# onecodex/needletail

Measured on AMD Instinct MI355X. Metric: Gbases/s canonical k=21 on 150 bp FASTQ; % HBM-read roofline at 1/2/4/8 GPU, higher is better.
Workload: dtype u64; 1 GPU; configs[1]: synthetic FASTQ 10M x 150 bp, k=21 canonical k-mers (normalize -> reverse_complement -> canonical_kmers), reduce mode, device-resident batch; reads_total=10000000, reads_this_gpu=10000000, read_len=150, k=21, seed=0x5eed0002, outputs=n_total,n_fwd,n_rc,4096-bin prefix histogram,sum64,xor64, parallelism=single GPU, rccl_ranks=0, devices_visible=1

## Files before the change

needletail_amd/csrc/ntk_api.hip:

```cpp
#include "../../include/needletail_amd.h"

#include <hip/hip_runtime.h>
#include <rccl/rccl.h>
#include <dlfcn.h>
#include <time.h>

#include <cstdlib>
#include <cstring>
#include <map>
#include <mutex>
#include <new>
#include <utility>
#include <thread>
#include <algorithm>
#include <vector>

#include "ntk_kernels.hpp"
#include "ntk_plan.hpp"
#include "ntk_compat_plan.hpp"

using namespace ntk;

const void *ntk_pick_scan2(int k, bool tie_rc, bool accept_u);
const void *ntk_pick_scan2_q(int k, bool canonical, bool tie_rc, bool accept_u);
// ... 301 lines not shown
    if (f.rearm_shards) c->work_dirty = false;
    return NTK_OK;
}

inline bool bad_device_input(const uint8_t *d_seq, const uint8_t *d_qual) { return !d_seq || ((uintptr_t)d_seq & 15) || ((uintptr_t)d_qual & 15); }

inline void scan_args_set_quality(ScanArgs &a, const uint8_t *d_qual, uint32_t cutoff)
{
    if (!cutoff) return;
    const QualityCut qc = quality_cut(cutoff);
    a.qual = d_qual; a.q_add = qc.add; a.q_sel = qc.sel;
}
template <class KernelQ, class Kernel, class... Args>
void launch_with_quality(ntk_ctx *c, KernelQ kernel_q, Kernel kernel, int blocks, int threads, const uint8_t *d_qual, uint32_t cutoff, Args... args)
{
    if (d_qual) {
        const QualityCut qc = quality_cut(cutoff);
        hipLaunchKernelGGL(kernel_q, dim3(blocks), dim3(threads), 0, c->stream, args..., d_qual, qc.add, qc.sel);
    } else
        hipLaunchKernelGGL(kernel, dim3(blocks), dim3(threads), 0, c->stream, args...);
}

inline int raw_bytes_blocks(const ntk_ctx *c, uint64_t n) { return blocks_for(c, n, (uint64_t)kPlThreads * 32, 8); }

template <bool WIDE> constexpr auto bytes_reduce_q = &canonical_bytes_reduce_kernel<WIDE, true, const uint8_t *, uint32_t, uint32_t>;
template <bool ACCEPT_U> constexpr auto wide_reduce_q = &wide_canonical_reduce_kernel<ACCEPT_U, true, const uint8_t *, uint32_t, uint32_t>;

void launch_raw_bytes(ntk_ctx *c, bool wide, int blocks, const uint8_t *d_seq, uint64_t n, uint32_t k, const uint32_t *run_if, bool normalized,
                      const uint8_t *d_qual, uint32_t cutoff)
{
    const uint32_t pb = k < 6 ? k : 6;
    launch_with_quality(c, wide ? bytes_reduce_q<true> : bytes_reduce_q<false>, wide ? &canonical_bytes_reduce_kernel<true> : &canonical_bytes_reduce_kernel<false>,
                        blocks, kPlThreads, d_qual, cutoff, d_seq, n, (n + 15) & ~(uint64_t)15, k, 2u * (k - pb), c->lut_complement(),
                        c->d_part_hist.p, c->d_part_scalars.p, run_if, wide && normalized ? 1u : 0u);
}

int run_bytes_reduce(ntk_ctx *c, const uint8_t *d_seq, uint64_t n, const ntk_params *p, bool zero_first, bool normalized,
                     const uint8_t *d_qual, uint32_t cutoff)
{
    const bool wide = p->k > 32, packed_first = wide && !(c->route_off & NTK_ROUTE_NO_SPECULATION);
    if (zero_first) HIPCHK(hipMemsetAsync(c->d_acc, 0, NTK_ACC_WORDS * sizeof(uint64_t), c->stream));
    const int blocks_raw = raw_bytes_blocks(c, n), blocks = packed_first ? blocks_for(c, n, kWkTile, 8) : blocks_raw;
    int rc = ensure_partials(c, blocks > blocks_raw ? blocks : blocks_raw);
    if (rc) return rc;
    Fold fold;
    fold.undigested = wide;
    TimedSpan span;
    if ((rc = span.begin(c))) return rc;
    if (packed_first) {
        const FlagPair f = next_flag(c);
        launch_with_quality(c, normalized ? wide_reduce_q<true> : wide_reduce_q<false>,
                            normalized ? &wide_canonical_reduce_kernel<true> : &wide_canonical_reduce_kernel<false>, blocks, kWkThreads, d_qual, cutoff,
                            d_seq, n, p->k, c->d_part_hist.p, c->d_part_scalars.p, f.flag, f.next);
        HIPCHK(hipGetLastError());
        fold.alt_flag = f.flag; fold.alt_rows = blocks_raw;
    }
    launch_raw_bytes(c, wide, blocks_raw, d_seq, n, p->k, fold.alt_flag, normalized, d_qual, cutoff);
    HIPCHK(hipGetLastError());
    if ((rc = span.end(c->ev_used))) return rc;
    return launch_fold(c, blocks, fold);
}

struct TileScan {
    const void *fn = nullptr;
    int threads = 0;
    size_t lds = 0;
    uint32_t stride = 0;
    uint64_t max_chunk = 0;
    int max_per_cu = 0;
    bool reduce = true;
    bool speculate = false;
    uint32_t cutoff = 0;
};
int launch_tile_scan(ntk_ctx *c, const TileScan &s, ScanArgs &a, bool zero_first)
{
    int per_cu = 0, rc = resident_blocks(c, s.fn, s.threads, s.lds, s.max_per_cu, &per_cu);
    if (rc) return rc;
    const uint64_t blocks_max = block_cap(c, per_cu), waves_per_block = (uint64_t)s.threads / 64;
    const uint64_t n = a.n_bytes;
    const int blocks_raw = s.speculate ? raw_bytes_blocks(c, n) : 0;
    a.n_tiles = tile_count(n, s.stride);
    a.work_counters = c->d_work.p;
    a.zero_words = NTK_ACC_WORDS;
    for (uint64_t tb = 0; tb < a.n_tiles; tb += kMaxTilesPerLaunch) {
        const LaunchPlan lp = plan_launch(n, s.stride, tb, blocks_max, waves_per_block, s.max_chunk);
        const int blocks = (int)lp.blocks;
        a.tile_begin = lp.tile_begin; a.tile_end = lp.tile_end;
        a.tail_tile_rel = lp.tail_tile_rel;
        a.n_shards = lp.n_shards;
        a.tiles_per_shard = lp.tiles_per_shard;
        a.chunk_tiles = lp.chunk_tiles;
        a.zero_acc = zero_first ? c->d_acc : nullptr;
        zero_first = false;
        if (c->work_dirty) HIPCHK(hipMemsetAsync(c->d_work.p, 0, kMaxShards * 64, c->stream));
        c->work_dirty = true;
        if (s.reduce) {
            if ((rc = ensure_partials(c, blocks > blocks_raw ? blocks : blocks_raw))) return rc;
            a.part_hist = c->d_part_hist.p; a.part_scalars = c->d_part_scalars.p;
        }
        Fold fold;
        fold.rearm_shards = a.n_shards;
        if (s.speculate) {
            const FlagPair f = next_flag(c);
            a.lower_flag = f.flag; a.lower_flag_next = f.next;
            fold.alt_flag = f.flag; fold.alt_rows = blocks_raw;
        }
        TimedSpan span;
        if ((rc = span.begin(c))) return rc;
        void *kargs[] = {(void *)&a};
        HIPCHK(hipLaunchKernel(s.fn, dim3(blocks), dim3(s.threads), kargs, s.lds, c->stream));
        if (s.speculate) {
            launch_raw_bytes(c, false, blocks_raw, a.seq, n, a.k, fold.alt_flag, false, a.qual, s.cutoff);
            HIPCHK(hipGetLastError());
        }
        if ((rc = span.end(c->ev_used))) return rc;
        if (s.reduce && (rc = launch_fold(c, blocks, fold))) return rc;
    }
    return NTK_OK;
}

int run_scan(ntk_ctx *c, const uint8_t *d_seq, uint64_t n, const ntk_params *p, const Mode &m, bool reduce,
             uint64_t *d_values, uint16_t *d_valid16, uint16_t *d_rc16, const uint8_t *d_qual = nullptr, const void *fused_min_fn = nullptr,
             uint32_t fused_w = 0)
{
    const bool zero_first = reduce && (p->flags & NTK_FLAG_RESET);
    if (n == 0) {
        if (zero_first) HIPCHK(hipMemsetAsync(c->d_acc, 0, NTK_ACC_WORDS * sizeof(uint64_t), c->stream));
        return NTK_OK;
    }
    if (bad_device_input(d_seq, d_qual)) return NTK_ERR_BAD_ARG;
    const uint32_t cutoff = d_qual ? quality_cutoff(p) : 0u;
    const uint32_t stride = !reduce ? (uint32_t)kTileStride : (p->k <= 32 ? (uint32_t)sv2_stride_bytes((int)(fused_w ? p->k + fused_w - 1 : p->k), fused_w == 0) : 0u);
    bool speculate = false;
    if (m.raw_bytes) {
        if (p->k > 32 && (!reduce || fused_min_fn)) return NTK_ERR_BAD_K;
        if (!reduce || fused_min_fn) return NTK_ERR_UNSUPPORTED;
        const uint8_t *qual = cutoff ? d_qual : nullptr;
        speculate = p->k <= 32 && tile_count(n, stride) <= kMaxTilesPerLaunch && !(c->route_off & NTK_ROUTE_NO_SPECULATION);
        if (!speculate) return run_bytes_reduce(c, d_seq, n, p, zero_first, m.accept_u, qual, cutoff);
    }
    const void *fn = fused_min_fn ? fused_min_fn : pick_scan(m, p->k, reduce, cutoff != 0);
    if (!fn) return NTK_ERR_BAD_ARG;
    int threads = !reduce ? 256 : (c->launch_threads ? c->launch_threads : 768);
    if (reduce && !c->launch_threads) {
        auto it = c->auto_threads.find(fn);
        if (it != c->auto_threads.end()) threads = it->second;
        else {
            int best_waves = 0;
            for (int t : {768, 640, 512}) {
                int blocks_cu = 0;
                HIPCHK(hipOccupancyMaxActiveBlocksPerMultiprocessor(&blocks_cu, fn, t, 0));
                if (blocks_cu > 2) blocks_cu = 2;
                if (blocks_cu * t > best_waves) { best_waves = blocks_cu * t; threads = t; }
            }
            c->auto_threads[fn] = threads;
        }
    }
    TileScan s;
    s.fn = fn; s.threads = threads; s.stride = stride; s.max_chunk = 24;
    s.lds = reduce ? 0 : (size_t)(threads / 64) * kStageWaveU64 * sizeof(uint64_t);
    s.max_per_cu = reduce ? 2 * (1024 / threads) : 4;
    s.reduce = reduce; s.speculate = speculate; s.cutoff = cutoff;
    ScanArgs a;
    memset(&a, 0, sizeof(a));
    scan_args_set_k(a, p->k);
    a.seq = d_seq; a.n_bytes = n;
    a.values = d_values; a.valid16 = d_valid16; a.rc16 = d_rc16;
    scan_args_set_quality(a, d_qual, cutoff);
    return launch_tile_scan(c, s, a, zero_first);
}

const void *pick_min_generic(const Mode &m, bool quality, bool f64, uint32_t k)
{
    const int kw = f64 ? 2 : m.kw;
// ... 1355 lines not shown
```

needletail_amd/csrc/ntk_kernels.hpp:

```cpp
#pragma once
#include <hip/hip_runtime.h>
#include <stdint.h>
#include <type_traits>

#include "ntk_tile.hpp"

namespace ntk {

typedef uint32_t u32x4 __attribute__((ext_vector_type(4)));

constexpr int kDppWaveShr1 = 0x138;
struct DevXL {
    __device__ __forceinline__ uint32_t prev_and(int s, uint32_t x, uint32_t mask) const { return prev(s, x) & mask; }
    __device__ __forceinline__ uint32_t prev_auto(uint32_t x) const { return prev(0, x); }
    __device__ __forceinline__ uint32_t prev(int, uint32_t x) const
    {
        return (uint32_t)__builtin_amdgcn_mov_dpp((int)x, kDppWaveShr1, 0xf, 0xf, true);
    }
    __device__ __forceinline__ uint32_t prev_add(int, uint32_t x, uint32_t c) const
    {
        uint32_t r;
        asm("s_nop 1\n v_add_u32_dpp %0, %1, %2 wave_shr:1 row_mask:0xf bank_mask:0xf bound_ctrl:1" : "=v"(r) : "v"(x), "v"(c));
        return r;
    }
    __device__ __forceinline__ uint32_t select_prev(int, bool take, uint32_t a, uint32_t b) const
    {
        uint32_t r;
        const uint64_t m = __builtin_amdgcn_ballot_w64(take);
        asm("s_nop 1\n s_mov_b64 vcc, %3\n v_cndmask_b32_dpp %0, %2, %1, vcc wave_shr:1 row_mask:0xf bank_mask:0xf bound_ctrl:1"
            : "=v"(r) : "v"(a), "v"(b), "s"(m) : "vcc");
        return r;
    }
};

template <int KW>
struct ReduceSink {
    uint64_t sum = 0, xr = 0;
    uint32_t n_fwd = 0, n_valid = 0;
    uint32_t *hist;
    uint32_t bin_shift;

    __device__ __forceinline__ void begin_tile(int64_t, uint32_t inval16, bool) { n_valid += __popc(~inval16 & 0xFFFFu); }
    __device__ __forceinline__ void emit(int, bool valid, bool take_fwd, uint32_t hi, uint32_t lo)
    {
        if (valid) {
            const uint64_t v = KW == 2 ? (((uint64_t)hi << 32) | lo) : (uint64_t)lo;
            sum += v;
            xr ^= v;
            n_fwd += take_fwd ? 1u : 0u;
            atomicAdd(&hist[KW == 2 ? (uint32_t)(v >> bin_shift) : (lo >> bin_shift)], 1u);
        }
    }
    __device__ __forceinline__ void end_tile() {}
};

constexpr int kStageRow = 18;
constexpr int kStageWaveU64 = kTileSlots * kStageRow;

template <int KW>
struct MaterializeSink {
    uint64_t *values;
    uint16_t *valid16, *rc16;
    uint64_t *stage;
    uint32_t lane = 0;
    int64_t base = 0;
    uint64_t n_bytes = 0;
    uint32_t inval = 0, rcbits = 0;
    bool halo = true;

    __device__ __forceinline__ void begin_tile(int64_t lane_base, uint32_t inval16, bool halo_lane) { base = lane_base; inval = inval16; rcbits = 0; halo = halo_lane; }
    __device__ __forceinline__ void emit(int j, bool, bool take_fwd, uint32_t hi, uint32_t lo)
    {
        if (values && !halo) stage[(lane - kHaloLanes) * kStageRow + j] = KW == 2 ? (((uint64_t)hi << 32) | lo) : (uint64_t)lo;
        rcbits |= (take_fwd ? 0u : 1u) << (15 - j);
    }
    __device__ __forceinline__ void end_tile()
    {
        if (!halo && base < (int64_t)n_bytes) {
            const uint32_t v = ~inval & 0xFFFFu;
            valid16[base >> 4] = (uint16_t)v;
            rc16[base >> 4] = (uint16_t)(rcbits & v);
        }
        if (!values) return;
        asm volatile("s_waitcnt lgkmcnt(0)" ::: "memory");
        const int64_t tile_pos0 = base - (int64_t)lane * 16 + kHaloLanes * 16;
        const int64_t limit = (int64_t)((n_bytes + 15) & ~(uint64_t)15);
#pragma unroll
        for (int s = 0; s < 8; s++) {
// ... 300 lines not shown
#undef NTK_R_BODY
#undef NTK_R_IN
#undef NTK_R_POS
    }

    template <bool WITH_BITS>
    __device__ __forceinline__ void region_plain(const int (&pos)[4], const uint32_t (&off)[4], const uint32_t (&w)[4], const uint32_t (&fb)[4])
    {
        uint64_t sd;
#define NTK_R_POS(i, BITS)                                                  \
        NTK_R_EXEC(i)                                                       \
        NTK_R_SUM_##i("%[w" #i "]")                                         \
        NTK_R_XOR("%[w" #i "]")                                             \
        BITS                                                                \
        NTK_R_HIST(i)
#define NTK_R_IN(i) [o##i] "v"(off[i]), [w##i] "v"(w[i]), [f##i] "v"(fb[i]), NTK_R_MASKS(i)
        if constexpr (WITH_BITS)
            asm volatile(NTK_R_POS(0, "v_add_u32 %[nfb], %[nfb], %[f0]\n") NTK_R_POS(1, "v_add_u32 %[nfb], %[nfb], %[f1]\n")
                         NTK_R_POS(2, "v_add_u32 %[nfb], %[nfb], %[f2]\n") NTK_R_POS(3, "v_add_u32 %[nfb], %[nfb], %[f3]\n") "s_mov_b64 exec, -1\n"
                         : [sumA] "+v"(sum), [sumB] "+v"(sum2), [xlo] "+v"(xlo), [nfb] "+v"(nf_bits), [sd] "=&s"(sd)
                         : NTK_R_IN(0), NTK_R_IN(1), NTK_R_IN(2), NTK_R_IN(3), [one] "v"(one) : "memory", "scc");
        else
            asm volatile(NTK_R_POS(0, "") NTK_R_POS(1, "") NTK_R_POS(2, "") NTK_R_POS(3, "") "s_mov_b64 exec, -1\n"
                         : [sumA] "+v"(sum), [sumB] "+v"(sum2), [xlo] "+v"(xlo), [sd] "=&s"(sd)
                         : NTK_R_IN(0), NTK_R_IN(1), NTK_R_IN(2), NTK_R_IN(3), [one] "v"(one) : "memory", "scc");
#undef NTK_R_IN
#undef NTK_R_POS
    }
    template <class S>
    __device__ __forceinline__ void emit_word_fwd(S &, const int (&pos)[4], const uint32_t (&v)[4])
    {
        const uint32_t off[4] = {word_cell(v[0]), word_cell(v[1]), word_cell(v[2]), word_cell(v[3])};
        region_plain<false>(pos, off, v, v);
    }
    template <class S>
    __device__ __forceinline__ void emit_min4(S &, const int (&pos)[4], const uint32_t (&cell4)[4], const uint32_t (&lo)[4], const uint32_t (&fb)[4])
    {
        uint32_t off[4];
#pragma unroll
        for (int i = 0; i < 4; i++) off[i] = HB == 14 ? cell4[i] : (cell4[i] >> 4) << 2;
        region_plain<true>(pos, off, lo, fb);
    }
    template <class S>
    __device__ __forceinline__ void emit_fwd(S &, const int (&pos)[4], const uint32_t (&T)[4], const uint32_t (&lo)[4])
    {
        if constexpr (kLight) {
            const uint32_t off[4] = {cell_offset_hi(T[0]), cell_offset_hi(T[1]), cell_offset_lo(T[2]), cell_offset_lo(T[3])};
            region_plain<false>(pos, off, lo, lo);
        } else {
            constexpr int SH = 64 - 2 * K;
            uint32_t hi[4], off[4];
            uint64_t sd;
#pragma unroll
            for (int i = 0; i < 4; i++) { hi[i] = SH ? T[i] >> SH : T[i]; off[i] = cell_offset_hi(T[i]); }
#define NTK_R_POS(i)                                                        \
        NTK_R_EXEC(i)                                                       \
        NTK_R_SUM_##i("%[l" #i "]")                                         \
        NTK_R_XOR("%[l" #i "]")                                             \
        "v_add_u32 %[sumh], %[sumh], %[h" #i "]\n"                           \
        "v_xor_b32 %[xh], %[xh], %[h" #i "]\n"                              \
        NTK_R_HIST(i)
#define NTK_R_IN(i) [o##i] "v"(off[i]), [l##i] "v"(lo[i]), [h##i] "v"(hi[i]), NTK_R_MASKS(i)
            asm volatile(NTK_R_POS(0) NTK_R_POS(1) NTK_R_POS(2) NTK_R_POS(3) "s_mov_b64 exec, -1\n"
                         : [sumA] "+v"(sum), [sumB] "+v"(sum2), [sumh] "+v"(sumh), [xlo] "+v"(xlo), [xh] "+v"(xh), [sd] "=&s"(sd)
                         : NTK_R_IN(0), NTK_R_IN(1), NTK_R_IN(2), NTK_R_IN(3), [one] "v"(one) : "memory", "scc");
#undef NTK_R_IN
#undef NTK_R_POS
        }
    }
#undef NTK_R_XOR
#undef NTK_R_SUM_3
#undef NTK_R_SUM_2
#undef NTK_R_SUM_1
#undef NTK_R_SUM_0
#undef NTK_R_CNT
#undef NTK_R_CNT_FIRST
#undef NTK_R_HIST
#undef NTK_R_MASKS
#undef NTK_R_EXEC
};

struct NoSink {};

#ifndef NTK_SV2_MINWAVES
#define NTK_SV2_MINWAVES 1
#endif
template <int K, bool TIE_RC, bool ACCEPT_U, bool QM = false, int HB = 12, int W = 0, bool FWD = false>
__global__ __launch_bounds__(1024, NTK_SV2_MINWAVES) void scan2_kernel(ScanArgs a)
{
    static_assert(K >= 1 && K <= 32 && (HB == 12 || HB == 14), "sv2 covers 1 <= k <= 32");
    static_assert(W == 0 || Sv2MinFused<K, W>::value, "fused minimizers: see ntk_tile.hpp");
    static_assert(W == 0 || K <= 16 || Sv2Light<K, HB>::value, "fused minimizers sum the lo word only: the cell must cover the bits above it");
    constexpr bool WORD = K <= 16;
    constexpr bool LIGHT = Sv2Light<K, HB>::value && !WORD;
    constexpr int kCells = 1 << HB;
    using Geo = Sv2Geom<(W ? K + W - 1 : K), (W == 0)>;
    constexpr uint32_t kStride = Geo::kStride, kHaloB = Geo::kHaloBytes;
    struct Lds { uint32_t hist[kCells]; uint64_t red[16 * 6]; };
    __shared__ Lds L;
    uint32_t *const s_hist = L.hist;
    uint64_t *const s_red = L.red;
    if ((uint32_t)(uintptr_t)&L.hist[0] != 0u) __builtin_trap();

    const uint32_t lane = threadIdx.x & 63u;
    const uint32_t wave = __builtin_amdgcn_readfirstlane(threadIdx.x >> 6);
    const uint32_t shard = blockIdx.x % a.n_shards;
    const uint32_t launch_tiles = (uint32_t)(a.tile_end - a.tile_begin);
    const uint32_t shard_begin = shard * a.tiles_per_shard;
    uint32_t shard_end = shard_begin + a.tiles_per_shard;
    if (shard_end > launch_tiles) shard_end = launch_tiles;
    uint32_t *ctr = a.work_counters + shard * 16;
    const uint32_t shard_tiles = shard_begin < shard_end ? shard_end - shard_begin : 0u;
    uint32_t next = 0;
    if (lane == 0) next = atomicAdd(ctr, a.chunk_tiles);
    if (a.zero_acc && blockIdx.x == 0)
        for (uint32_t i = threadIdx.x; i < a.zero_words; i += blockDim.x) a.zero_acc[i] = 0;
    for (int i = threadIdx.x; i < kCells / 4; i += blockDim.x) reinterpret_cast<u32x4 *>(s_hist)[i] = u32x4{0u, 0u, 0u, 0u};
    __syncthreads();
    constexpr bool SPEC = TIE_RC && !ACCEPT_U && W == 0 && !FWD;
    uint32_t lc = 0;
    if (SPEC && a.lower_flag_next && blockIdx.x == 0 && threadIdx.x == 0) *a.lower_flag_next = 0;
    DevXL xl;
    DevMasks2<K, HB> mp;
    NoSink sink;
    mp.rep = lane & (uint32_t)(DevMasks2<K, HB>::kWordCopies - 1);

    next = __builtin_amdgcn_readfirstlane(next);
    while (next < shard_tiles) {
        const uint32_t r0 = shard_begin + next;
        uint32_t r1 = r0 + a.chunk_tiles;
        if (r1 > shard_end) r1 = shard_end;
        if (lane == 0) next = atomicAdd(ctr, a.chunk_tiles);
        const uint64_t t0 = a.tile_begin + r0;
        const uint64_t run_byte = t0 * kStride;
        const uint32_t halo = t0 ? kHaloB : 0u;
        const uint64_t cbase = (uint64_t)a.seq + run_byte - halo;
        uint64_t rem = ((a.n_bytes + 15) & ~(uint64_t)15) - (run_byte - halo);
        if (rem > 0xFFFFFF00ull) rem = 0xFFFFFF00ull;
        const uint32_t blo = __builtin_amdgcn_readfirstlane((uint32_t)cbase);
        const uint32_t bhi = __builtin_amdgcn_readfirstlane((uint32_t)(cbase >> 32));
        const uint32_t nrec = __builtin_amdgcn_readfirstlane((uint32_t)rem);
        __amdgpu_buffer_rsrc_t rs = __builtin_amdgcn_make_buffer_rsrc((void *)(((uint64_t)bhi << 32) | blo), 0, nrec, 0x00020000);
        __amdgpu_buffer_rsrc_t rq = rs;
        if constexpr (QM) {
            const uint64_t qbase = (uint64_t)a.qual + run_byte - halo;
            const uint32_t qlo = __builtin_amdgcn_readfirstlane((uint32_t)qbase);
            const uint32_t qhi = __builtin_amdgcn_readfirstlane((uint32_t)(qbase >> 32));
            rq = __builtin_amdgcn_make_buffer_rsrc((void *)(((uint64_t)qhi << 32) | qlo), 0, nrec, 0x00020000);
        }
        uint32_t voff = lane * 16u - (kHaloB - halo);
        uint64_t tile_byte = run_byte;
        auto load_tile = [&](uint32_t off) { return __builtin_amdgcn_raw_buffer_load_b128(rs, off, 0, 0); };
        auto load_qual = [&](uint32_t off) { return __builtin_amdgcn_raw_buffer_load_b128(rq, off, 0, 0); };
        auto process = [&](const u32x4 &t, const u32x4 &q, uint32_t r, auto &&after_encode) {
            const bool tail = r >= a.tail_tile_rel;
            Raw16 raw{t.x, t.y, t.z, t.w};
            if constexpr (SPEC && !QM) {
                if (tail) lc |= or_of_input_bytes(raw, (int64_t)a.n_bytes - ((int64_t)tile_byte - (int64_t)kHaloB + lane * 16));
                else lc = bitop3<0xFE>(bitop3<0xFE>(lc, t.x, t.y), t.z, t.w);
            }
            if constexpr (QM) raw = quality_break16(raw, Raw16{q.x, q.y, q.z, q.w}, a.q_add, a.q_sel);
            if constexpr (SPEC && QM) {
                if (tail) lc |= or_of_input_bytes(lower_watch16(raw), (int64_t)a.n_bytes - ((int64_t)tile_byte - (int64_t)kHaloB + lane * 16));
                else lc = lower_watch_or(lower_watch_or(lower_watch_or(lower_watch_or(lc, raw.x), raw.y), raw.z), raw.w);
            }
            const EncSV2 en = encode16_sv2<ACCEPT_U>(raw);
            mp.template compute<(W ? K + W - 1 : K), (W == 0)>(en, tail, (int64_t)tile_byte - (int64_t)kHaloB + lane * 16, a.n_bytes);
            after_encode();
            if constexpr (W > 0) lane_tile_sv2_min<TIE_RC, K, W>(sink, xl, mp, en.code, en.rcode);
            else if constexpr (WORD) lane_tile_sv2w<TIE_RC, K, FWD>(sink, xl, mp, en.code, en.rcode);
            else if constexpr (FWD) lane_tile_sv2_fwd<K>(sink, xl, mp, en.code);
            else lane_tile_sv2<TIE_RC, K>(sink, xl, mp, en.code, en.rcode);
            voff += kStride; tile_byte += kStride;
        };
        auto load_first = [&](__amdgpu_buffer_rsrc_t r_, uint32_t off) {
            uint32_t d[4];
#pragma unroll
            for (int i = 0; i < 4; i++) {
                const int32_t o = (int32_t)off + 4 * i;
                const uint32_t v = __builtin_amdgcn_raw_buffer_load_b32(r_, o >= 0 ? (uint32_t)o : 0u, 0, 0);
                d[i] = o >= 0 ? v : 0u;
            }
            return u32x4{d[0], d[1], d[2], d[3]};
        };
        const bool split_first = kHaloB % 16u != 0u && t0 == 0;
        u32x4 ta = split_first ? load_first(rs, voff) : load_tile(voff), qa = ta;
        if constexpr (QM) qa = split_first ? load_first(rq, voff) : load_qual(voff);
        for (uint32_t r = r0; r < r1; r++)
            process(ta, qa, r, [&] {
                if (r + 1 < r1) { ta = load_tile(voff + kStride); if constexpr (QM) qa = load_qual(voff + kStride); }
            });
        next = __builtin_amdgcn_readfirstlane(next);
    }

    if constexpr (SPEC)
        if (a.lower_flag && __builtin_amdgcn_ballot_w64((lc & 0x20202020u) != 0u) != 0ull && lane == 0) atomicOr(a.lower_flag, 1u);
    asm volatile("s_waitcnt lgkmcnt(0)" ::: "memory");
    uint64_t sum = mp.sum + mp.sum2 + ((uint64_t)mp.sumh << 32);
    uint64_t xr = (WORD || LIGHT) ? (uint64_t)mp.xlo : ((uint64_t)mp.xh << 32) | mp.xlo, nf, nv = 0;
    uint64_t shi = 0, xf = 0;
    uint32_t *ph = a.part_hist + (size_t)blockIdx.x * kHistBins;
    nf = lane == 0 ? mp.nf_s : 0u;
    if constexpr (W > 0) nf = mp.nf_bits;
    __syncthreads();
    constexpr int HBE = HB;
    for (int c = threadIdx.x; c < kHistBins; c += blockDim.x) {
        uint32_t tot = 0;
        if constexpr (K <= 6) {
            if (c < (1 << (2 * K)))
                for (int r = 0; r < DevMasks2<K, HB>::kWordCopies; r++) tot += s_hist[(r << (2 * K)) + c];
        } else
#pragma unroll
        for (int q = 0; q < kCells / kHistBins; q++) {
            const uint32_t f = c * (kCells / kHistBins) + q, h = s_hist[f];
            tot += h;
            if constexpr (LIGHT) {
                const uint32_t pfx = f >> (HB - HBE);
                shi += (uint64_t)(pfx >> (32 + HBE - 2 * K)) * h;
                xf ^= (h & 1u) ? pfx : 0u;
            }
        }
        ph[c] = tot; nv += tot;
    }
    if constexpr (LIGHT) {
        constexpr uint32_t low_mask = 2 * K - HBE >= 32 ? 0xFFFFFFFFu : ((1u << ((2 * K - HBE) & 31)) - 1u);
        sum += shi << 32;
        xr = (xf << (2 * K - HBE)) | (uint64_t)(mp.xlo & low_mask);
    }
#pragma unroll
    for (int o = 32; o > 0; o >>= 1) {
        sum += __shfl_xor(sum, o, 64);
        xr ^= __shfl_xor(xr, o, 64);
        nf += __shfl_xor(nf, o, 64);
        nv += __shfl_xor(nv, o, 64);
    }
    if (lane == 0) { s_red[wave * 4 + 0] = nv; s_red[wave * 4 + 1] = nf; s_red[wave * 4 + 2] = sum; s_red[wave * 4 + 3] = xr; }
    __syncthreads();
    if (threadIdx.x == 0) {
        uint64_t tv = 0, tf = 0, ts = 0, tx = 0;
        for (uint32_t w = 0; w < (blockDim.x >> 6); w++) {
            tv += s_red[w * 4 + 0]; tf += s_red[w * 4 + 1]; ts += s_red[w * 4 + 2]; tx ^= s_red[w * 4 + 3];
        }
        uint64_t *ps = a.part_scalars + (size_t)blockIdx.x * 4;
        if constexpr (W > 0 && !TIE_RC) tf = tv - tf;
        if constexpr (FWD) tf = tv;
        if constexpr (WORD && K < 16 && W == 0) { ts >>= 32 - 2 * K; tx >>= 32 - 2 * K; }
        ps[0] = tv; ps[1] = tf; ps[2] = ts; ps[3] = tx;
    }
}

#ifndef NTK_SCAN_TEMPLATES_ONLY
#ifndef NTK_MINGEN_WAVES_F64
#define NTK_MINGEN_WAVES_F64 4
#endif
#ifndef NTK_MINGEN_WAVES_G
#define NTK_MINGEN_WAVES_G 4
#endif
constexpr int min_gen_waves(bool f64) { return f64 ? NTK_MINGEN_WAVES_F64 : NTK_MINGEN_WAVES_G; }
constexpr int min_gen_threads(bool f64) { return min_gen_waves(f64) == 3 ? 768 : 512; }
struct DevMinOut {
    uint64_t sum = 0, sum2 = 0;
    uint32_t sumh = 0, xh = 0;
    uint32_t xlo = 0, nfb = 0, one = 1;
    template <bool WIDE>
    __device__ __forceinline__ void region(const uint64_t *V, const uint32_t (&off)[4], const uint32_t (&lo)[4], const uint32_t (&hi)[4],
                                           const uint32_t (&sb)[4])
    {
        uint64_t sd;
#define NTK_M_POS(i, ACC, W)                                                \
        "s_mov_b64 exec, %[m" #i "]\n"                                      \
        "v_mad_u64_u32 %[" ACC "], %[sd], %[l" #i "], 1, %[" ACC "]\n"       \
        "v_xor_b32 %[xlo], %[xlo], %[l" #i "]\n"                            \
        "v_add_u32 %[nfb], %[nfb], %[f" #i "]\n"                            \
        W                                                                   \
        "ds_add_u32 %[o" #i "], %[one]\n"
// ... 1134 lines not shown
```

needletail_amd/csrc/ntk_plan.hpp:

```cpp
#pragma once
#include <stdint.h>

namespace ntk {

constexpr int kMaxShards = 256;
constexpr uint64_t kMaxTilesPerLaunch = (uint64_t)8 << 22;

inline uint64_t tile_count(uint64_t n, uint64_t stride) { return (n + stride - 1) / stride; }

struct LaunchPlan {
    uint64_t tile_begin, tile_end;
    uint32_t chunk_tiles;
    uint32_t blocks;
    uint32_t n_shards;
    uint32_t tiles_per_shard;
    uint32_t tail_tile_rel;
};

inline LaunchPlan plan_launch(uint64_t n, uint64_t stride, uint64_t tile_begin, uint64_t blocks_max, uint64_t waves_per_block, uint64_t max_chunk)
{
    LaunchPlan p;
    const uint64_t n_tiles = tile_count(n, stride);
    p.tile_begin = tile_begin;
    p.tile_end = tile_begin + kMaxTilesPerLaunch < n_tiles ? tile_begin + kMaxTilesPerLaunch : n_tiles;
    const uint64_t tiles = p.tile_end - p.tile_begin;
    uint64_t chunk = tiles / (blocks_max * waves_per_block * 4);
    chunk = chunk < 1 ? 1 : (chunk > max_chunk ? max_chunk : chunk);
    const uint64_t want_blocks = (tiles + chunk * waves_per_block - 1) / (chunk * waves_per_block);
    p.blocks = (uint32_t)(want_blocks < blocks_max ? want_blocks : blocks_max);
    p.chunk_tiles = (uint32_t)chunk;
    p.n_shards = p.blocks < (uint32_t)kMaxShards ? (p.blocks ? p.blocks : 1u) : (uint32_t)kMaxShards;
    p.tiles_per_shard = (uint32_t)((tiles + p.n_shards - 1) / p.n_shards);
    const uint64_t first_tail = n / stride;
    p.tail_tile_rel = first_tail < tile_begin ? 0u : (first_tail - tile_begin > 0xFFFFFFFEull ? 0xFFFFFFFFu : (uint32_t)(first_tail - tile_begin));
    return p;
}

}
```

needletail_amd/csrc/ntk_tile.hpp:

```cpp
#pragma once
#include <stdint.h>

#if defined(__HIPCC__)
#define NTK_HD __host__ __device__ __forceinline__
#else
#define NTK_HD inline
#endif

namespace ntk {

constexpr int kTileBytes = 1024;
constexpr int kHistBins = 4096;

struct ScanArgs {
    const uint8_t *seq;
    uint64_t n_bytes;
    uint64_t n_tiles;
    uint64_t tile_begin;
    uint64_t tile_end;
    uint32_t *work_counters;
    uint32_t n_shards;
    uint32_t tiles_per_shard;
    uint32_t chunk_tiles;
    uint32_t tail_tile_rel;
    uint32_t k;
    uint32_t sh_r;
    uint32_t mask_hi;
    uint32_t mask_lo;
    uint32_t smear[5];
    uint32_t bin_shift;
    uint32_t *part_hist;
    uint64_t *part_scalars;
    uint64_t *values;
    uint16_t *valid16;
    uint16_t *rc16;
    const uint8_t *qual;
    uint32_t q_add, q_sel;
    uint64_t *zero_acc;
    uint32_t zero_words;
    uint32_t *lower_flag, *lower_flag_next;
    uint32_t min_w, min_halo_lanes;
    uint32_t min_smear[6];
    uint32_t min_overlap;
    uint32_t min_smear_kw[6];
};

inline void scan_args_set_k(ScanArgs &a, uint32_t k)
{
    a.k = k;
    if (k > 16) {
        a.sh_r = 64 - 2 * k;
        a.mask_hi = k == 32 ? 0xFFFFFFFFu : ((1u << (2 * k - 32)) - 1u);
        a.mask_lo = 0xFFFFFFFFu;
    } else {
        a.sh_r = 32 - 2 * k;
        a.mask_hi = 0;
        a.mask_lo = k == 16 ? 0xFFFFFFFFu : ((1u << (2 * k)) - 1u);
    }
    uint32_t len = 1;
    for (int i = 0; i < 5; i++) {
        uint32_t s = len < k ? (len < k - len ? len : k - len) : 0;
        a.smear[i] = s;
        len += s;
    }
    const uint32_t p = k < 6 ? k : 6;
    a.bin_shift = 2 * (k - p);
}

template <int TT>
NTK_HD uint32_t bitop3(uint32_t a, uint32_t b, uint32_t c)
{
#if defined(__HIP_DEVICE_COMPILE__)
    return __builtin_amdgcn_bitop3_b32(a, b, c, TT);
#else
    uint32_t r = 0;
    for (int i = 0; i < 8; i++)
        if ((TT >> i) & 1) r |= ((i & 4) ? a : ~a) & ((i & 2) ? b : ~b) & ((i & 1) ? c : ~c);
    return r;
#endif
}
NTK_HD uint32_t bfi(uint32_t mask, uint32_t a, uint32_t b) { return bitop3<0xCA>(mask, a, b); }
NTK_HD uint32_t and_or(uint32_t a, uint32_t b, uint32_t c) { return bitop3<0xEA>(a, b, c); }
NTK_HD uint32_t or_and(uint32_t a, uint32_t b, uint32_t c) { return bitop3<0xA8>(a, b, c); }

NTK_HD uint32_t perm(uint32_t hi, uint32_t lo, uint32_t sel)
{
#if defined(__HIP_DEVICE_COMPILE__)
    return __builtin_amdgcn_perm(hi, lo, sel);
#else
    const uint64_t src = ((uint64_t)hi << 32) | lo;
    uint32_t r = 0;
    for (int i = 0; i < 4; i++) {
        const uint32_t s = (sel >> (8 * i)) & 0xFF;
        const uint32_t b = s < 8 ? (uint32_t)((src >> (8 * s)) & 0xFF) : (s >= 13 ? 0xFFu : 0u);
        r |= b << (8 * i);
    }
    return r;
#endif
}

NTK_HD uint32_t alignbit(uint32_t hi, uint32_t lo, uint32_t sh)
{
#if defined(__HIP_DEVICE_COMPILE__)
    return __builtin_amdgcn_alignbit(hi, lo, sh);
#else
    return (uint32_t)(((((uint64_t)hi) << 32) | lo) >> (sh & 31));
// ... 967 lines not shown
```

Baseline: 3307 Gbases/s.

## Use ticket-based guided chunk scheduling with per-shard buffer descriptor and cross-chunk prefetch

Work distribution changes from atomically adding chunk_tiles to a counter to pulling one-step tickets. Each ticket maps to a big chunk at first and to chunks a third that size for the last two fifths of a shard, which is meant to balance the tail across waves. The buffer descriptor is now built once per shard instead of once per chunk, and the first tile of the next chunk is prefetched while the current chunk finishes, so chunk boundaries no longer stall the load pipeline. Launches are split so that a shard always fits in one descriptor; this adds planning complexity and more atomic traffic from the smaller chunks.

```diff
diff --git a/needletail_amd/csrc/ntk_api.hip b/needletail_amd/csrc/ntk_api.hip
--- a/needletail_amd/csrc/ntk_api.hip
+++ b/needletail_amd/csrc/ntk_api.hip
@@ -407,14 +407,15 @@
     a.n_tiles = tile_count(n, s.stride);
     a.work_counters = c->d_work.p;
     a.zero_words = NTK_ACC_WORDS;
-    for (uint64_t tb = 0; tb < a.n_tiles; tb += kMaxTilesPerLaunch) {
-        const LaunchPlan lp = plan_launch(n, s.stride, tb, blocks_max, waves_per_block, s.max_chunk);
+    for (uint64_t tb = 0; tb < a.n_tiles;) {
+        const LaunchPlan lp = plan_bounded_launch(n, s.stride, tb, blocks_max, waves_per_block, s.max_chunk);
+        tb = lp.tile_end;
         const int blocks = (int)lp.blocks;
         a.tile_begin = lp.tile_begin; a.tile_end = lp.tile_end;
         a.tail_tile_rel = lp.tail_tile_rel;
         a.n_shards = lp.n_shards;
         a.tiles_per_shard = lp.tiles_per_shard;
-        a.chunk_tiles = lp.chunk_tiles;
+        a.chunk_tiles = lp.chunk_tiles; a.chunk_small = lp.chunk_small; a.n_big = lp.n_big;
         a.zero_acc = zero_first ? c->d_acc : nullptr;
         zero_first = false;
         if (c->work_dirty) HIPCHK(hipMemsetAsync(c->d_work.p, 0, kMaxShards * 64, c->stream));
diff --git a/needletail_amd/csrc/ntk_kernels.hpp b/needletail_amd/csrc/ntk_kernels.hpp
--- a/needletail_amd/csrc/ntk_kernels.hpp
+++ b/needletail_amd/csrc/ntk_kernels.hpp
@@ -4,6 +4,7 @@
 #include <type_traits>
 
 #include "ntk_tile.hpp"
+#include "ntk_plan.hpp"
 
 namespace ntk {
 
@@ -470,6 +471,13 @@
 
 struct NoSink {};
 
+__device__ __forceinline__ uint32_t pull_ticket(uint32_t *ctr)
+{
+    uint32_t zero = 0;
+    asm volatile("" : "+v"(zero));
+    return atomicAdd((uint32_t *)((char *)ctr + zero), 1u);
+}
+
 #ifndef NTK_SV2_MINWAVES
 #define NTK_SV2_MINWAVES 1
 #endif
@@ -500,7 +508,7 @@
     uint32_t *ctr = a.work_counters + shard * 16;
     const uint32_t shard_tiles = shard_begin < shard_end ? shard_end - shard_begin : 0u;
     uint32_t next = 0;
-    if (lane == 0) next = atomicAdd(ctr, a.chunk_tiles);
+    if (lane == 0) next = pull_ticket(ctr);
     if (a.zero_acc && blockIdx.x == 0)
         for (uint32_t i = threadIdx.x; i < a.zero_words; i += blockDim.x) a.zero_acc[i] = 0;
     for (int i = threadIdx.x; i < kCells / 4; i += blockDim.x) reinterpret_cast<u32x4 *>(s_hist)[i] = u32x4{0u, 0u, 0u, 0u};
@@ -513,31 +521,29 @@
     NoSink sink;
     mp.rep = lane & (uint32_t)(DevMasks2<K, HB>::kWordCopies - 1);
 
-    next = __builtin_amdgcn_readfirstlane(next);
-    while (next < shard_tiles) {
-        const uint32_t r0 = shard_begin + next;
-        uint32_t r1 = r0 + a.chunk_tiles;
-        if (r1 > shard_end) r1 = shard_end;
-        if (lane == 0) next = atomicAdd(ctr, a.chunk_tiles);
-        const uint64_t t0 = a.tile_begin + r0;
-        const uint64_t run_byte = t0 * kStride;
-        const uint32_t halo = t0 ? kHaloB : 0u;
-        const uint64_t cbase = (uint64_t)a.seq + run_byte - halo;
-        uint64_t rem = ((a.n_bytes + 15) & ~(uint64_t)15) - (run_byte - halo);
-        if (rem > 0xFFFFFF00ull) rem = 0xFFFFFF00ull;
-        const uint32_t blo = __builtin_amdgcn_readfirstlane((uint32_t)cbase);
-        const uint32_t bhi = __builtin_amdgcn_readfirstlane((uint32_t)(cbase >> 32));
-        const uint32_t nrec = __builtin_amdgcn_readfirstlane((uint32_t)rem);
-        __amdgpu_buffer_rsrc_t rs = __builtin_amdgcn_make_buffer_rsrc((void *)(((uint64_t)bhi << 32) | blo), 0, nrec, 0x00020000);
-        __amdgpu_buffer_rsrc_t rq = rs;
-        if constexpr (QM) {
-            const uint64_t qbase = (uint64_t)a.qual + run_byte - halo;
-            const uint32_t qlo = __builtin_amdgcn_readfirstlane((uint32_t)qbase);
-            const uint32_t qhi = __builtin_amdgcn_readfirstlane((uint32_t)(qbase >> 32));
-            rq = __builtin_amdgcn_make_buffer_rsrc((void *)(((uint64_t)qhi << 32) | qlo), 0, nrec, 0x00020000);
-        }
-        uint32_t voff = lane * 16u - (kHaloB - halo);
-        uint64_t tile_byte = run_byte;
+    const uint64_t shard_tile0 = a.tile_begin + shard_begin;
+    const uint32_t halo0 = shard_tile0 ? kHaloB : 0u;
+    const uint64_t anchor = shard_tile0 * kStride - halo0, padded_end = (a.n_bytes + 15) & ~(uint64_t)15;
+    uint64_t rem = anchor < padded_end ? padded_end - anchor : 0u;
+    if (rem > 0xFFFFFF00ull) rem = 0xFFFFFF00ull;
+    const uint64_t cbase = (uint64_t)a.seq + anchor;
+    const uint32_t blo = __builtin_amdgcn_readfirstlane((uint32_t)cbase);
+    const uint32_t bhi = __builtin_amdgcn_readfirstlane((uint32_t)(cbase >> 32));
+    const uint32_t nrec = __builtin_amdgcn_readfirstlane((uint32_t)rem);
+    const __amdgpu_buffer_rsrc_t rs = __builtin_amdgcn_make_buffer_rsrc((void *)(((uint64_t)bhi << 32) | blo), 0, nrec, 0x00020000);
+    __amdgpu_buffer_rsrc_t rq = rs;
+    if constexpr (QM) {
+        const uint64_t qbase = (uint64_t)a.qual + anchor;
+        const uint32_t qlo = __builtin_amdgcn_readfirstlane((uint32_t)qbase);
+        const uint32_t qhi = __builtin_amdgcn_readfirstlane((uint32_t)(qbase >> 32));
+        rq = __builtin_amdgcn_make_buffer_rsrc((void *)(((uint64_t)qhi << 32) | qlo), 0, nrec, 0x00020000);
+    }
+    const uint32_t soff0 = halo0 - kHaloB;
+    const uint32_t lane_id = lane;
+    {
+        uint32_t lane = lane_id;
+        uint32_t voff = 0;
+        uint64_t tile_byte = 0;
         auto load_tile = [&](uint32_t off) { return __builtin_amdgcn_raw_buffer_load_b128(rs, off, 0, 0); };
         auto load_qual = [&](uint32_t off) { return __builtin_amdgcn_raw_buffer_load_b128(rq, off, 0, 0); };
         auto process = [&](const u32x4 &t, const u32x4 &q, uint32_t r, auto &&after_encode) {
@@ -571,14 +577,36 @@
             }
             return u32x4{d[0], d[1], d[2], d[3]};
         };
-        const bool split_first = kHaloB % 16u != 0u && t0 == 0;
-        u32x4 ta = split_first ? load_first(rs, voff) : load_tile(voff), qa = ta;
-        if constexpr (QM) qa = split_first ? load_first(rq, voff) : load_qual(voff);
-        for (uint32_t r = r0; r < r1; r++)
-            process(ta, qa, r, [&] {
-                if (r + 1 < r1) { ta = load_tile(voff + kStride); if constexpr (QM) qa = load_qual(voff + kStride); }
-            });
         next = __builtin_amdgcn_readfirstlane(next);
+        TileChunk ch = ticket_chunk(next, shard_tiles, a.chunk_tiles, a.n_big, a.chunk_small);
+        u32x4 ta = u32x4{0u, 0u, 0u, 0u}, qa = ta;
+        if (ch.begin < ch.end) {
+            const bool split_first = kHaloB % 16u != 0u && shard_tile0 + ch.begin == 0;
+            voff = lane * 16u + (soff0 + ch.begin * kStride);
+            ta = split_first ? load_first(rs, voff) : load_tile(voff);
+            if constexpr (QM) qa = split_first ? load_first(rq, voff) : load_qual(voff);
+        }
+        while (ch.begin < ch.end) {
+            asm volatile("" : "+v"(lane));
+            if (lane == 0) next = pull_ticket(ctr);
+            const uint32_t r0 = shard_begin + ch.begin, r1 = shard_begin + ch.end;
+            tile_byte = (a.tile_begin + r0) * kStride;
+            TileChunk nx = ch;
+            for (uint32_t r = r0; r < r1; r++)
+                process(ta, qa, r, [&] {
+                    bool more = r + 1 < r1;
+                    uint32_t step = kStride;
+                    if (!more) {
+                        next = __builtin_amdgcn_readfirstlane(next);
+                        nx = ticket_chunk(next, shard_tiles, a.chunk_tiles, a.n_big, a.chunk_small);
+                        more = nx.begin < nx.end;
+                        step = (shard_begin + nx.begin - r) * kStride;
+                    }
+                    if (more) { ta = load_tile(voff + step); if constexpr (QM) qa = load_qual(voff + step); }
+                });
+            ch = nx;
+            voff = lane * 16u + (soff0 + ch.begin * kStride);
+        }
     }
 
     if constexpr (SPEC)
diff --git a/needletail_amd/csrc/ntk_plan.hpp b/needletail_amd/csrc/ntk_plan.hpp
--- a/needletail_amd/csrc/ntk_plan.hpp
+++ b/needletail_amd/csrc/ntk_plan.hpp
@@ -1,28 +1,53 @@
 #pragma once
 #include <stdint.h>
+
+#if defined(__HIPCC__)
+#define NTK_PLAN_HD __host__ __device__ __forceinline__
+#else
+#define NTK_PLAN_HD inline
+#endif
 
 namespace ntk {
 
 constexpr int kMaxShards = 256;
 constexpr uint64_t kMaxTilesPerLaunch = (uint64_t)8 << 22;
+constexpr uint64_t kMaxTilesPerShard = (uint64_t)1 << 22;
+static_assert(kMaxTilesPerShard * 1008 + 48 + 1024 < 0xFFFFFF00ull, "a shard must fit one buffer descriptor");
 
 inline uint64_t tile_count(uint64_t n, uint64_t stride) { return (n + stride - 1) / stride; }
 
 struct LaunchPlan {
     uint64_t tile_begin, tile_end;
     uint32_t chunk_tiles;
+    uint32_t chunk_small;
+    uint32_t n_big;
     uint32_t blocks;
     uint32_t n_shards;
     uint32_t tiles_per_shard;
     uint32_t tail_tile_rel;
 };
 
-inline LaunchPlan plan_launch(uint64_t n, uint64_t stride, uint64_t tile_begin, uint64_t blocks_max, uint64_t waves_per_block, uint64_t max_chunk)
+struct TileChunk { uint32_t begin, end; };
+NTK_PLAN_HD TileChunk ticket_chunk(uint32_t ticket, uint32_t shard_tiles, uint32_t c_big, uint32_t n_big, uint32_t c_small)
+{
+    const uint32_t t = ticket < shard_tiles ? ticket : shard_tiles;
+    const uint32_t big = t < n_big ? t : n_big;
+    TileChunk c;
+    c.begin = big * c_big + (t - big) * c_small;
+    c.end = c.begin + (t < n_big ? c_big : c_small);
+    if (c.end > shard_tiles) c.end = shard_tiles;
+    return c;
+}
+
+constexpr uint32_t kSmallDiv = 3, kTailNum = 2, kTailDen = 5;
+
+inline LaunchPlan plan_launch(uint64_t n, uint64_t stride, uint64_t tile_begin, uint64_t blocks_max, uint64_t waves_per_block, uint64_t max_chunk,
+                              uint64_t launch_tiles = kMaxTilesPerLaunch)
 {
     LaunchPlan p;
     const uint64_t n_tiles = tile_count(n, stride);
     p.tile_begin = tile_begin;
-    p.tile_end = tile_begin + kMaxTilesPerLaunch < n_tiles ? tile_begin + kMaxTilesPerLaunch : n_tiles;
+    p.tile_end = tile_begin + launch_tiles < n_tiles ? tile_begin + launch_tiles : n_tiles;
     const uint64_t tiles = p.tile_end - p.tile_begin;
     uint64_t chunk = tiles / (blocks_max * waves_per_block * 4);
     chunk = chunk < 1 ? 1 : (chunk > max_chunk ? max_chunk : chunk);
@@ -31,9 +56,19 @@
     p.chunk_tiles = (uint32_t)chunk;
     p.n_shards = p.blocks < (uint32_t)kMaxShards ? (p.blocks ? p.blocks : 1u) : (uint32_t)kMaxShards;
     p.tiles_per_shard = (uint32_t)((tiles + p.n_shards - 1) / p.n_shards);
+    p.chunk_small = p.chunk_tiles < kSmallDiv ? p.chunk_tiles : p.chunk_tiles / kSmallDiv;
+    const uint32_t all_big = (p.tiles_per_shard + p.chunk_tiles - 1) / p.chunk_tiles;
+    p.n_big = p.chunk_small == p.chunk_tiles ? all_big : (uint32_t)((uint64_t)p.tiles_per_shard * (kTailDen - kTailNum) / kTailDen / p.chunk_tiles);
     const uint64_t first_tail = n / stride;
     p.tail_tile_rel = first_tail < tile_begin ? 0u : (first_tail - tile_begin > 0xFFFFFFFEull ? 0xFFFFFFFFu : (uint32_t)(first_tail - tile_begin));
     return p;
 }
 
+inline LaunchPlan plan_bounded_launch(uint64_t n, uint64_t stride, uint64_t tile_begin, uint64_t blocks_max, uint64_t waves_per_block, uint64_t max_chunk)
+{
+    const LaunchPlan p = plan_launch(n, stride, tile_begin, blocks_max, waves_per_block, max_chunk);
+    if (p.tiles_per_shard <= kMaxTilesPerShard) return p;
+    return plan_launch(n, stride, tile_begin, blocks_max, waves_per_block, max_chunk, (uint64_t)p.n_shards * kMaxTilesPerShard);
 }
+
+}
diff --git a/needletail_amd/csrc/ntk_tile.hpp b/needletail_amd/csrc/ntk_tile.hpp
--- a/needletail_amd/csrc/ntk_tile.hpp
+++ b/needletail_amd/csrc/ntk_tile.hpp
@@ -22,6 +22,8 @@
     uint32_t n_shards;
     uint32_t tiles_per_shard;
     uint32_t chunk_tiles;
+    uint32_t chunk_small;
+    uint32_t n_big;
     uint32_t tail_tile_rel;
     uint32_t k;
     uint32_t sh_r;
```

Result: no change. 3329 Gbases/s, median of 5 (+0.7%).
